# lmjakt/kmer_spans

Measured on AMD Instinct MI355X. Metric: Gbases/sec scanned (k=13, log-ratio score) at 1/2/4/8 MI355X; spans bit-exact, higher is better.
Workload: dtype f64

## Files before the change

kmer_spans_amd/csrc/ks_scan_chunked.hip:

```cpp
#include <hip/hip_fp16.h>
#include <hipcub/hipcub.hpp>

#include <algorithm>
#include <cstring>
#include <type_traits>
#include <vector>

#include "ks_scan_common.h"

namespace ks {

ks_status launch_scan_lane(ks_ctx *ctx, const uint8_t *seq, int64_t total, const int64_t *ra, const int64_t *rb,
                           const int32_t *rs, int64_t n, int k, const TableView &tv, uint64_t mw,
                           double min_score, uint32_t *visits, const RegionBuf &out,
                           const unsigned long long *d_cnt = nullptr, int64_t segcap = 0,
                           const ScanMode &mode = ScanMode(), int init_step = 1, const int64_t *offs = nullptr,
                           const uint32_t *packed = nullptr, hipStream_t strm = nullptr);

namespace {

constexpr int CH = 256;
constexpr int NB = 16;
constexpr int kModeClean = 0, kModeL = 1, kModeR = 2, kModeU = 3;

// ... 1434 lines not shown
  __shared__ __attribute__((aligned(16))) uint32_t s_esc[(BS / 64) * 2 * 64];
  __shared__ double s_lut[kLineLutMax];
  for (int i = threadIdx.x; i < tv.nlut; i += BS) s_lut[i] = tv.lut[i];
  __syncthreads();
  const int lane = threadIdx.x & 63, wv = threadIdx.x >> 6;
  const int64_t c = g.c0 + (int64_t)blockIdx.x * BS + threadIdx.x;
  if (c - lane >= g.nch) return;
  const bool live = c < g.nch;
  const int64_t start = live ? g.start[c] : (int64_t)k;
  const int n = live ? g.n[c] : 0;
  const bool first = live && (c == 0 || g.run[c - 1] != g.run[c]);
  const uint32_t kmask = (1u << (2 * k)) - 1u;
  P1Lane<!kExact, kTrlr, kExact> L;
  L.init(start, n, first, live, (live && xh) ? xh[c] : 0.0);
  LaneBases B;
  B.load(g.packed, total, start - k);
  const int kx = k + J - 1;
  const uint64_t xmask = (1ull << (2 * kx)) - 1ull;
  uint64_t x = B.first_key(kx);
  const double first_val = (kTrlr && first) ? ec.ks[(uint32_t)(x >> (2 * (J - 1))) & kmask] : 0.0;

  uint8_t *const ring = s_ring + wv * 4096;
  uint32_t *const esc = s_esc + wv * 128;
  const uint32_t ring_lds = __builtin_amdgcn_readfirstlane(lds_addr(ring));
  const uint32_t esc_lds = __builtin_amdgcn_readfirstlane(lds_addr(esc));
  const uint8_t *__restrict__ lines = tv.line;
  auto dwords = [&](uint64_t xk) -> uint32_t {
    const uint32_t c1 = (uint32_t)(xk >> 4) & 3u, c2 = (uint32_t)(xk >> 2) & 3u, c3 = (uint32_t)xk & 3u;
    const uint32_t d2 = (13u * (OWN + 4 + 4 * c1 + c2)) >> 5, d3 = (B3 + 11u * (16 * c1 + 4 * c2 + c3)) >> 5;
    return d2 | (d3 << 8);
  };
  auto issue = [&](uint64_t xk, int slot) {
    const uint32_t idx = (uint32_t)(xk >> 6), dd = dwords(xk);
    const int j = lane & 7;
#pragma unroll
    for (int q = 0; q < 8; ++q) {
      const int ow = 8 * q + (lane >> 3);
      const uint32_t li = (uint32_t)__shfl((int)idx, ow);
      const uint32_t od = (uint32_t)__shfl((int)dd, ow);
      const uint32_t d2 = od & 0xffu, d3 = od >> 8;
      const uint32_t dw = j < NO ? (uint32_t)j
                                 : (j < NO + 2 ? d2 + (uint32_t)(j - NO)
                                               : (j < NO + 4 ? min(d3 + (uint32_t)(j - NO - 2), 31u) : 0u));
      glds4(lines + (size_t)li * 128 + dw * 4, ring_lds + (uint32_t)(slot * 2048 + q * 256));
    }
  };
  double vp[J];
  uint64_t xp = 0;
  bool ep = false;
  constexpr int KW = kc_words(J);
  uint32_t *const kcl = kStore ? kc + kc_slot(live ? c : g.c0, 0, J) : nullptr;
  uint32_t recp[KW] = {};
  auto process = [&](int sp_, const double *vv, uint64_t xk, bool e) {
    double v5 = vv[J - 1];
    uint32_t c5 = 0;
    if (e) {
      const uint32_t pr = esc[(sp_ & 1) * 64 + lane];
      const uint32_t km = (uint32_t)xk & kmask;
      c5 = (km & 1u) ? (pr >> 16) : (pr & 0xffffu);
      v5 = s_lut[c5];
    }
    if constexpr (kStore) {
      uint32_t rec[KW];
#pragma unroll
      for (int q = 0; q < KW; ++q) rec[q] = recp[q];
      rec[(J - 1) / 2] |= c5 << (16 * ((J - 1) & 1));
      if (live) kc_store<KW>(kcl + (size_t)sp_ * 64 * KW, rec);
    }
#pragma unroll
    for (int t = 0; t < J; ++t) {
      const int i = sp_ * J + t;
      if (i < n) {
        double sv = t == J - 1 ? v5 : vv[t];
        if (kTrlr && first && i == 0) sv = first_val;
        if (visits) atomicAdd(&visits[(uint32_t)(xk >> (2 * (J - 1 - t))) & kmask], 1u);
        L.step(sv, i, ec, cand);
      }
    }
  };
  uint64_t x1 = 0, x2 = 0;
  issue(x, 0);
  x1 = B.next_key(x, J, xmask);
  issue(x1, 1);
  for (int st = 0; st < NS; ++st) {
    const uint64_t xs = x;
    if constexpr (kStore) {
      if (st + 1 >= NS) asm volatile("s_waitcnt vmcnt(1)" ::: "memory");
      else if (st >= 2) asm volatile("s_waitcnt vmcnt(9)" ::: "memory");
      else asm volatile("s_waitcnt vmcnt(8)" ::: "memory");
    } else {
      if (st + 1 < NS) asm volatile("s_waitcnt vmcnt(8)" ::: "memory");
      else asm volatile("s_waitcnt vmcnt(0)" ::: "memory");
    }
    const uint8_t *ln = ring + (st & 1) * 2048 + lane * 32;
    double v[J];
    uint32_t rec[KW] = {};
    bool e = false;
    {
      const uint4 q0 = *reinterpret_cast<const uint4 *>(ln);
      const uint4 q1 = *reinterpret_cast<const uint4 *>(ln + 16);
      const uint32_t D[8] = {q0.x, q0.y, q0.z, q0.w, q1.x, q1.y, q1.z, q1.w};
      const uint64_t lo = (uint64_t)D[0] | ((uint64_t)D[1] << 32);
      const uint64_t hi = (uint64_t)D[2] | (NO > 3 ? ((uint64_t)D[3] << 32) : 0ull);
      auto f13 = [&](int b) -> uint32_t {
        const uint64_t w = b < 64 ? ((lo >> b) | (b > 51 ? (hi << (64 - b)) : 0ull)) : (hi >> (b - 64));
        return (uint32_t)w & 0x1fffu;
      };
      const uint32_t c1 = (uint32_t)(xs >> 4) & 3u, c2 = (uint32_t)(xs >> 2) & 3u, c3 = (uint32_t)xs & 3u;
      uint32_t cs[J];
#pragma unroll
      for (int t = 0; t < OWN; ++t) cs[t] = f13(13 * t);
      const uint32_t l0 = f13(13 * OWN), l1 = f13(13 * (OWN + 1)), l2 = f13(13 * (OWN + 2)),
                     l3 = f13(13 * (OWN + 3));
      cs[OWN] = c1 == 0 ? l0 : (c1 == 1 ? l1 : (c1 == 2 ? l2 : l3));
      const uint32_t b2 = 13u * (OWN + 4 + 4 * c1 + c2), b3 = B3 + 11u * (16 * c1 + 4 * c2 + c3);
      cs[OWN + 1] = (uint32_t)(((uint64_t)D[NO] | ((uint64_t)D[NO + 1] << 32)) >> (b2 & 31)) & 0x1fffu;
      const uint32_t c11 = (uint32_t)(((uint64_t)D[NO + 2] | ((uint64_t)D[NO + 3] << 32)) >> (b3 & 31)) & 0x7ffu;
      e = c11 == 0x7ffu;
      cs[OWN + 2] = e ? 0u : c11;
#pragma unroll
      for (int t = 0; t < J; ++t) v[t] = s_lut[cs[t]];
      if constexpr (kStore) kc_pack<J>(cs, rec);
    }
    {
      const uint32_t km = (uint32_t)xs & kmask;
      const uint16_t *src = e ? tv.codes + (km & ~1u) : tv.codes;
      glds4(src, esc_lds + (uint32_t)((st & 1) * 256));
    }
    x = x1;
    if (st + 2 < NS) {
      x2 = B.next_key(x1, J, xmask);
      asm volatile("s_waitcnt lgkmcnt(0)" ::: "memory");
      issue(x2, st & 1);
      x1 = x2;
    }
    if (st > 0) process(st - 1, vp, xp, ep);
#pragma unroll
    for (int t = 0; t < J; ++t) vp[t] = v[t];
    if constexpr (kStore) {
#pragma unroll
      for (int q = 0; q < KW; ++q) recp[q] = rec[q];
    }
    xp = xs;
    ep = e;
  }
  if constexpr (kStore) asm volatile("s_waitcnt vmcnt(1)" ::: "memory");
  else asm volatile("s_waitcnt vmcnt(0)" ::: "memory");
  process(NS - 1, vp, xp, ep);
  if (!live) return;
  if constexpr (kExact) L.finish_exact(c, g, o, cr, xh, err);
  else L.finish(c, o, sp);
}

constexpr int kCodeBlock = 1024;
constexpr int kCodeDepth = 2;

__device__ __forceinline__ uint32_t packed_kmer(const uint32_t *__restrict__ packed, int64_t total, int64_t p0, int k) {
  const int64_t w0 = p0 >> 4, wlast = total >> 4;
  const uint64_t x = ((uint64_t)packed[min(w0, wlast)] << 32) | packed[min(w0 + 1, wlast)];
  const int sk = (int)(p0 & 15);
  return (uint32_t)(x >> (64 - 2 * (sk + k))) & ((1u << (2 * k)) - 1u);
}

template <int J, bool kTrlr, bool kVisits>
__global__ void __launch_bounds__(kCodeBlock) k_pass1c(Chunks g, int64_t total, int k, TableView tv, EmitCfg ec,
                                                       uint32_t *__restrict__ visits, P1 o, Cand cand,
                                                       const double *__restrict__ xh, Carry cr,
                                                       unsigned int *__restrict__ err,
                                                       const uint32_t *__restrict__ kc) {
  constexpr int NS = kc_steps(J), W = kc_words(J), D = kCodeDepth;
  constexpr int NG = (NS + D - 1) / D;
  extern __shared__ double s_clut[];
  for (int i = threadIdx.x; i < tv.nlut; i += kCodeBlock) s_clut[i] = tv.lut[i];
  __syncthreads();
  const int64_t c = g.c0 + (int64_t)blockIdx.x * kCodeBlock + threadIdx.x;
  if (c >= g.nch) return;
  const int64_t start = g.start[c];
  const int n = g.n[c];
  const bool first = c == 0 || g.run[c - 1] != g.run[c];
  const uint32_t kmask = (1u << (2 * k)) - 1u;
  const uint32_t *__restrict__ rp = kc + kc_slot(c, 0, J);
  uint32_t cur[D][W] = {}, nxt[D][W] = {};
  auto fetch = [&](int gi, uint32_t (&b)[D][W]) {
#pragma unroll
    for (int d = 0; d < D; ++d)
      if (gi * D + d < NS) kc_load<W>(rp + (size_t)(gi * D + d) * 64 * W, b[d]);
  };
  fetch(0, cur);
  P1Lane<false, kTrlr, true> L;
  L.init(start, n, first, true, xh[c]);
  double first_val = 0.0;
  if ((kTrlr && first) || (c & 63) == 0) {
    const uint32_t km0 = packed_kmer(g.packed, total, start - k, k);
    if (kTrlr && first) first_val = ec.ks[km0];
    if ((c & 63) == 0 && (cur[0][0] & 0xffffu) != (uint32_t)tv.codes[km0]) atomicOr(err, 128u);
  }
  LaneBases B;
  uint64_t x = 0;
  const uint64_t xmask = (1ull << (2 * (k + J - 1))) - 1ull;
  if (kVisits) {
    B.load(g.packed, total, start - k);
    x = B.first_key(k + J - 1);
  }
  for (int gi = 0; gi < NG; ++gi) {
    if (gi + 1 < NG) fetch(gi + 1, nxt);
    if (gi * D * J < n) {
#pragma unroll
      for (int d = 0; d < D; ++d) {
        const int st = gi * D + d;
        if (st < NS) {
#pragma unroll
          for (int t = 0; t < J; ++t) {
            const int i = st * J + t;
            if (i < n) {
              const uint32_t code = (cur[d][t >> 1] >> (16 * (t & 1))) & 0xffffu;
              double sv = s_clut[code];
              if (kTrlr && first && i == 0) sv = first_val;
              if (kVisits) atomicAdd(&visits[(uint32_t)(x >> (2 * (J - 1 - t))) & kmask], 1u);
              L.step(sv, i, ec, cand);
            }
          }
          if (kVisits) x = B.next_key(x, J, xmask);
        }
      }
    }
#pragma unroll
    for (int d = 0; d < D; ++d)
#pragma unroll
      for (int q = 0; q < W; ++q) cur[d][q] = nxt[d][q];
  }
  L.finish_exact(c, g, o, cr, xh, err);
}

__global__ void __launch_bounds__(256) k_test_codes(uint32_t *__restrict__ kc, Chunks g, Carry cr, int64_t nch,
                                                    int J, int what, unsigned int *__restrict__ err) {
  auto spoil = [&](int64_t c, int i) {
    uint32_t *p = kc + kc_slot(c, i / J, J) + (size_t)((i % J) >> 1);
    const int sh = 16 * ((i % J) & 1);
    const uint32_t code = (*p >> sh) & 0xffffu;
    *p = (*p & ~(0xffffu << sh)) | ((code ? 0u : 1u) << sh);
  };
  if (what == 1) {
    for (int64_t c = threadIdx.x; c < nch; c += blockDim.x)
      for (int i = 0; i < CH; ++i) spoil(c, i);
  } else if (what == 0) {
    if (threadIdx.x == 0) spoil(0, 0);
  } else {
    __shared__ unsigned long long s_first;
    if (threadIdx.x == 0) s_first = ~0ull;
    __syncthreads();
    for (int64_t c = threadIdx.x; c < nch; c += blockDim.x)
      if ((c & 63) != 0 && g.n[c] > 1 && c + 1 < nch && g.run[c + 1] == g.run[c] && cr.mode[c] != kModeClean &&
          cr.hq[c] < 0)
        atomicMin(&s_first, (unsigned long long)c);
    __syncthreads();
    if (threadIdx.x == 0) {
      if (s_first == ~0ull) atomicOr(err, 256u);
      else spoil((int64_t)s_first, 1);
    }
  }
}

constexpr int kRankBlock = 768;

template <int OWN>
__global__ void __launch_bounds__(kRankBlock) k_pass1r(Chunks g, int64_t total, int k, TableView tv, EmitCfg ec,
                                                       uint32_t *__restrict__ visits, P1 o, Cand cand) {
  constexpr int BS = kRankBlock;
  constexpr int J = OWN + 2;
  constexpr int NS = (CH + J - 1) / J;
  static_assert(OWN + 2 <= 8, "own, L1, L2 dwords in 8 lanes");
  __shared__ __attribute__((aligned(16))) uint8_t s_ring[(BS / 64) * 2 * 2048];
  __shared__ unsigned long long s_pc[2 * kRankPieceLds];
  const int nl = min(tv.nrpc, kRankPieceLds);
  for (int i = threadIdx.x; i < 2 * nl; i += BS) s_pc[i] = tv.rpc[i];
  __syncthreads();
  const int lane = threadIdx.x & 63, wv = threadIdx.x >> 6;
  const int64_t c = g.c0 + (int64_t)blockIdx.x * BS + threadIdx.x;
  if (c - lane >= g.nch) return;
  const bool live = c < g.nch;
  const int64_t start = live ? g.start[c] : (int64_t)k;
  const int n = live ? g.n[c] : 0;
  const bool first = live && (c == 0 || g.run[c - 1] != g.run[c]);
  const uint32_t kmask = (1u << (2 * k)) - 1u;
  P1Lane<false, false> L;
  L.init(start, n, first, live, 0.0);
  LaneBases B;
  B.load(g.packed, total, start - k);
  const int kx = k + J - 1;
  const uint64_t xmask = (1ull << (2 * kx)) - 1ull;
  uint64_t x = B.first_key(kx);
  uint8_t *const ring = s_ring + wv * 4096;
  const uint32_t ring_lds = __builtin_amdgcn_readfirstlane(lds_addr(ring));
  const uint8_t *__restrict__ lines = tv.rline;
  const unsigned long long *__restrict__ gpc = tv.rpc;
  const double thr = tv.rthr;
  auto issue = [&](uint64_t xk, int slot) {
    const uint32_t idx = (uint32_t)(xk >> 4);
    const uint32_t c1 = (uint32_t)(xk >> 2) & 3u, c2 = (uint32_t)xk & 3u;
    const uint32_t dd = (OWN + c1) | ((OWN + 4 + 4 * c1 + c2) << 8);
    const int j = lane & 7;
#pragma unroll
    for (int q = 0; q < 8; ++q) {
      const int ow = 8 * q + (lane >> 3);
      const uint32_t li = (uint32_t)__shfl((int)idx, ow);
      const uint32_t od = (uint32_t)__shfl((int)dd, ow);
      const uint32_t dw = j < OWN ? (uint32_t)j : (j == OWN ? (od & 0xffu) : (j == OWN + 1 ? (od >> 8) : 0u));
      glds4(lines + (size_t)li * 128 + dw * 4, ring_lds + (uint32_t)(slot * 2048 + q * 256));
    }
  };
  auto decode = [&](uint32_t code) -> double {
    const uint32_t p = code >> kRankOffBits;
    const unsigned long long off = code & ((1u << kRankOffBits) - 1u);
    unsigned long long base, inc;
    if ((int)p < nl) {
      base = s_pc[2 * p];
      inc = s_pc[2 * p + 1];
    } else {
      base = gpc[2 * p];
      inc = gpc[2 * p + 1];
    }
    return __longlong_as_double((long long)(base + off * inc)) - thr;
  };
  double vp[J];
  uint64_t xp = 0;
  auto process = [&](int sp_, const double *vv, uint64_t xk) {
#pragma unroll
    for (int t = 0; t < J; ++t) {
      const int i = sp_ * J + t;
      if (i < n) {
        if (visits) atomicAdd(&visits[(uint32_t)(xk >> (2 * (J - 1 - t))) & kmask], 1u);
        L.step(vv[t], i, ec, cand);
      }
    }
  };
  uint64_t x1 = 0, x2 = 0;
  issue(x, 0);
  x1 = B.next_key(x, J, xmask);
  issue(x1, 1);
  for (int st = 0; st < NS; ++st) {
    const uint64_t xs = x;
    if (st + 1 < NS) asm volatile("s_waitcnt vmcnt(8)" ::: "memory");
    else asm volatile("s_waitcnt vmcnt(0)" ::: "memory");
    const uint8_t *ln = ring + (st & 1) * 2048 + lane * 32;
    uint32_t cs[J];
    {
      const uint4 q0 = *reinterpret_cast<const uint4 *>(ln);
      const uint4 q1 = *reinterpret_cast<const uint4 *>(ln + 16);
      const uint32_t D[8] = {q0.x, q0.y, q0.z, q0.w, q1.x, q1.y, q1.z, q1.w};
#pragma unroll
      for (int t = 0; t < J; ++t) cs[t] = D[t];
    }
    x = x1;
    if (st + 2 < NS) {
      x2 = B.next_key(x1, J, xmask);
      asm volatile("s_waitcnt lgkmcnt(0)" ::: "memory");
      issue(x2, st & 1);
      x1 = x2;
    }
    if (st > 0) process(st - 1, vp, xp);
#pragma unroll
    for (int t = 0; t < J; ++t) vp[t] = decode(cs[t]);
    xp = xs;
  }
  asm volatile("s_waitcnt vmcnt(0)" ::: "memory");
  process(NS - 1, vp, xp);
  if (live) L.finish(c, o, SummP1{});
}

constexpr int kLdsTableK = 7;
__global__ void __launch_bounds__(1024) k_pass1_lds_int(Chunks g, int64_t total, int k, TableView tv, EmitCfg ec,
                                                        uint32_t *__restrict__ visits, P1 o, Cand cand) {
  __shared__ int32_t s_val[1 << (2 * kLdsTableK)];
  const int nk = 1 << (2 * k);
  for (int i = threadIdx.x; i < nk; i += blockDim.x) s_val[i] = (int32_t)tv_get(tv, (uint32_t)i);
  __syncthreads();
  const uint32_t kmask = (uint32_t)nk - 1u;
  for (int64_t c = g.c0 + (int64_t)blockIdx.x * blockDim.x + threadIdx.x; c < g.nch;
       c += (int64_t)gridDim.x * blockDim.x) {
    const int64_t start = g.start[c];
    const int n = g.n[c];
    const int64_t q0 = start - k;
    Window16 win(g.packed, total, q0);
    int32_t prev = 0, best = 0, asum = 0, pmin = INT32_MAX, pmax = INT32_MIN;
    int beg = -1, arg = 0, parg = 0;
// ... 1960 lines not shown
  int32_t *se = cv.take<int32_t>(nch);
  long long *sD = cv.take<long long>(nch * 6);
  int32_t *sA = cv.take<int32_t>(nch * 2);
  double *x = cv.take<double>(nch);
  uint8_t *cmode = cv.take<uint8_t>(nch);
  int32_t *hq = cv.take<int32_t>(nch * 2);
  double *hmax = cv.take<double>(nch);
  unsigned long long *cnts = cv.take<unsigned long long>(5 * kSegs + 8);
  uint8_t *flag = cv.take<uint8_t>(nch + 64);
  char *xa0 = cv.take<char>(ntiles * 32), *xa1 = cv.take<char>(ntiles * 32);
  double *pa = cv.take<double>(nch);
  double *pb = cv.take<double>(nch);
  uint8_t *pz = cv.take<uint8_t>(nch);
  int32_t *spe = cv.take<int32_t>(nch * 2);
  long long *spd = cv.take<long long>(nch * 6);
  int32_t *spa = cv.take<int32_t>(nch * 2);
  unsigned long long *nfix = cv.take<unsigned long long>(nch + 2);
  uint8_t *ssel = cv.take<uint8_t>(nch);
  double2 *tagg = cv.take<double2>(ntiles);
  double *tin = cv.take<double>(ntiles);
  const int64_t ngt = nch / 64 + 2;
  int32_t *gte = cv.take<int32_t>(ngt);
  long long *gtd = cv.take<long long>(ngt * 6);
  long long *gtm = cv.take<long long>(ngt);
  int32_t *gtee = cv.take<int32_t>(ngt);
  const int64_t rcap_h = std::max<int64_t>(65536, nch / 128);
  int32_t *rslot = cv.take<int32_t>(nch);
  int64_t *rchunk = cv.take<int64_t>(2 * rcap_h);
  unsigned long long *rcnt = cv.take<unsigned long long>(8);
  double *rval = cv.take<double>(2 * rcap_h * 256);
  *bytes = cv.off;

  Work w{};
  if (!base) return w;
  w.g = Chunks{kp.start, kp.n, kp.run, nch, packed};
  w.p1 = P1{p1d, p1d + nch, p1d + 2 * nch, p1d + 3 * nch, p1d + 4 * nch, p1d + 5 * nch, p1i, p1i + nch, spec,
            p1i + 2 * nch};
  w.p1.ep = ep;
  w.sm = Summ{se, sD, sD + 2 * nch, sD + 4 * nch, sA};
  w.cr = Carry{x, cmode, hq, hmax, hq + nch};
  w.cnts = cnts;
  w.flag = flag;
  auto xtiles = [&](char *p) {
    return XTiles{reinterpret_cast<int32_t *>(p), reinterpret_cast<int32_t *>(p) + ntiles,
                  reinterpret_cast<long long *>(p + ntiles * 8), reinterpret_cast<long long *>(p + ntiles * 16),
                  reinterpret_cast<double *>(p + ntiles * 24)};
  };
  w.xagg = xtiles(xa0);
  w.xtin = xtiles(xa1);
  w.pa = pa;
  w.pb = pb;
  w.pz = pz;
  w.sp1 = SummP1{spe, spd, spd + 2 * nch, spd + 4 * nch, spa};
  w.nfix = nfix;
  w.fix = reinterpret_cast<int64_t *>(nfix + 2);
  w.tagg = tagg;
  w.tin = tin;
  w.trun = kp.trun;
  w.tcomp = TileComp{gte, gtd, gtd + 2 * ngt, gtd + 4 * ngt, gtm, gtee};
  w.rpb = ReplayBuf{plan.p1summ ? rslot : nullptr, rchunk, rval, rcnt, rcap_h};
  if (plan.p1summ) {
    w.sm.sel = ssel;
    w.sm.pD = w.sp1.D;
    w.sm.pM = w.sp1.M;
    w.sm.pN = w.sp1.N;
    w.sm.pA = w.sp1.A;
  }
  w.nwin = (nch + 63) / 64;
  return w;
}

struct ScanCall {
  ks_ctx *ctx;
  const ks_dev_seqs *s;
  int64_t total;
  int k;
  const TableView &tv;
  const EmitCfg ec;
  const Runs &runs;
  const RunLayout &lay;
  const RegionBuf &rb;
  uint32_t *visits, *visits_rescan;
  const ScanMode &mode;
};

Chunks view(const Chunks &g, const Half &h) {
  Chunks v = g;
  v.c0 = h.c0;
  v.nch = h.c1;
  return v;
}

constexpr int kWpb = 2;

ks_status ascan(const ScanCall &c, const Work &w, const P1 &o, double *out, const Half &h, hipStream_t strm) {
  const int64_t nruns = c.runs.n;
  if (h.r1 <= h.r0) return KS_OK;
  const dim3 gr((unsigned)(h.r1 - h.r0));
  if (h.t1 <= h.t0) return launch(k_approx_scan, gr, dim3(64), 0, strm, c.lay.cbase, h.r1, o, out, h.r0);
  const dim3 g4((unsigned)((h.t1 - h.t0 + kWpb - 1) / kWpb)), b4(64 * kWpb);
  KS_TRY(launch(k_ascan_tiles, g4, b4, 0, strm, c.lay.tbase, c.lay.cbase, nruns, w.trun, o, w.tagg, h.t0, h.t1));
  KS_TRY(launch(k_ascan_runs, gr, dim3(64), 0, strm, c.lay.tbase, h.r1, w.tagg, w.tin, h.r0));
  return launch(k_ascan_apply, g4, b4, 0, strm, c.lay.tbase, c.lay.cbase, nruns, w.trun, o, w.tin, out, h.t0, h.t1);
}

ks_status predict(const ScanCall &c, const Work &w, const Half &h, hipStream_t strm) {
  P1 pp = w.p1;
  pp.asum = w.pa;
  pp.cexit = w.pb;
  pp.special = w.pz;
  KS_HIP(hipMemsetAsync(w.pz + h.c0, 0, (size_t)(h.c1 - h.c0), strm));
  const size_t lds = (size_t)2 << (2 * c.tv.approx_k);
  const int per_cu = lds <= ((size_t)32 << 10) ? 4 : 1;
  const unsigned gl = (unsigned)std::max<int64_t>(
      1, std::min<int64_t>((h.c1 - h.c0 + 1023) / 1024, (int64_t)c.ctx->num_cus * per_cu));
  KS_HIP(hipFuncSetAttribute((const void *)k_predict<4>, hipFuncAttributeMaxDynamicSharedMemorySize, (int)lds));
  KS_TRY(launch(k_predict<4>, dim3(gl), dim3(1024), lds, strm, view(w.g, h), c.total, c.k, c.tv.approx,
                c.tv.approx_k, pp.asum, pp.cexit));
  return ascan(c, w, pp, w.xh, h, strm);
}

ks_status pass1_half(const ScanCall &c, const ScanPlan &plan, const Work &w, const Half &h, hipStream_t strm,
                     const Cand &cand) {
  const Chunks gv = view(w.g, h);
  const int64_t n = h.c1 - h.c0;
  const TableView &tv = c.tv;
  const EmitCfg &ec = c.ec;
  const P1 &p1 = w.p1;
  const SummP1 &sp1 = w.sp1;
  const double *xh = plan.entry_reuse ? w.cr.x : (plan.p1summ ? w.xh : nullptr);
  const Carry &cr = w.cr;
  unsigned int *err = reinterpret_cast<unsigned int *>(w.cnts + 2 * kSegs + 2 * (&h - plan.half) + 1);
  const bool trlr = ec.trlr != 0;
  auto blocks = [&](int64_t per) { return dim3((unsigned)((n + per - 1) / per)); };
  auto persistent = [&](int per_cu) {
    return dim3((unsigned)std::max<int64_t>(1, std::min<int64_t>((n + 1023) / 1024, (int64_t)per_cu * c.ctx->num_cus)));
  };
  switch (plan.family) {
    case P1Family::Lds:
      if (trlr)
        return launch(k_pass1_lds<true>, persistent(1), dim3(1024), 0, strm, gv, c.total, c.k, tv, ec, c.visits, p1,
                      cand, xh, sp1);
      if (plan.exact)
        return launch(k_pass1_lds_int, persistent(2), dim3(1024), 0, strm, gv, c.total, c.k, tv, ec, c.visits, p1,
                      cand);
      return launch(k_pass1_lds<false>, persistent(1), dim3(1024), 0, strm, gv, c.total, c.k, tv, ec, c.visits, p1,
                    cand, xh, sp1);
    case P1Family::Line: {
      const int own = tv.line_own;
      if (plan.codes_read)
        return pick_int<5, 7, 4>(plan.codes_J, [&](auto j) {
          return pick_bool(trlr, [&](auto t) {
            return pick_bool(c.visits != nullptr, [&](auto v) {
              return launch(k_pass1c<decltype(j)::value, decltype(t)::value, decltype(v)::value>, blocks(kCodeBlock),
                            dim3(kCodeBlock), (size_t)tv.nlut * 8, strm, gv, c.total, c.k, tv, ec, c.visits, p1, cand,
                            xh, cr, err, w.kc);
            });
          });
        });
      if (tv.rline && !trlr && !plan.p1summ && own == 3)
        return launch(k_pass1r<3>, blocks(kRankBlock), dim3(kRankBlock), 0, strm, gv, c.total, c.k, tv, ec, c.visits,
                      p1, cand);
      if (tv.line_kind == 3)
        return pick_wide_own(own, [&](auto o) {
          return pick_bool(trlr, [&](auto t) {
            return pick_int<1, 2, 0>(plan.entry_reuse ? (plan.codes_write ? 2 : 1) : 0, [&](auto x) {
              return launch(k_pass1w<decltype(o)::value, decltype(t)::value, (decltype(x)::value > 0),
                                     (decltype(x)::value > 1)>,
                            blocks(kWideBlock), dim3(kWideBlock), 0, strm, gv, c.total, c.k, tv, ec, c.visits, p1, cand,
                            xh, sp1, cr, err, w.kc);
            });
          });
        });
      if (!plan.comp)
        return pick_int<3, 4, 2>(own, [&](auto o) {
          return pick_bool(trlr, [&](auto t) {
            return launch(k_pass1l<decltype(o)::value, true, false, decltype(t)::value>, blocks(1024), dim3(1024), 0,
                          strm, gv, c.total, c.k, tv, ec, c.visits, p1, cand, xh, sp1, cr, err, w.kc);
          });
        });
      return pick_u16_own(own, [&](auto o) {
        return pick_bool(tv.nlut <= kLineLutMax, [&](auto l) {
          return pick_bool(trlr, [&](auto t) {
            return pick_int<1, 2, 0>(plan.entry_reuse ? (plan.codes_write ? 2 : 1) : 0, [&](auto x) {
              return launch(k_pass1l<decltype(o)::value, false, decltype(l)::value, decltype(t)::value,
                                     (decltype(x)::value > 0), (decltype(x)::value > 1 && decltype(l)::value)>,
                            blocks(768), dim3(768), 0, strm, gv, c.total, c.k, tv, ec, c.visits, p1, cand, xh, sp1, cr,
                            err, w.kc);
            });
          });
        });
      });
    }
    case P1Family::F64Expanded:
      return pick_int<3, 4, 2>(plan.J, [&](auto j) {
        return pick_bool(trlr, [&](auto t) {
          return launch(k_pass1pf<decltype(j)::value, decltype(t)::value, 512>, blocks(512), dim3(512), 0, strm, gv,
                        c.s->seq, c.total, c.k, tv, ec, c.visits, p1, cand, c.runs.packed, xh, sp1);
        });
      });
    case P1Family::CompExpanded:
      return pick_int<3, 5, 2>(plan.J, [&](auto j) {
        return pick_bool(plan.lds_lut, [&](auto l) {
          return pick_bool(trlr, [&](auto t) {
            return launch(k_pass1p<decltype(j)::value, decltype(l)::value, decltype(t)::value>, blocks(kP1Block),
                          dim3(kP1Block), 0, strm, gv, c.s->seq, c.total, c.k, tv, ec, c.visits, p1, cand,
                          c.runs.packed, xh, sp1);
          });
        });
      });
    case P1Family::Plain:
      break;
  }
  return fail(KS_ERR_INTERNAL, "chunked scan: no pass-1 launch per half for this table form");
}

ks_status pass1_tail(const ScanCall &c, const ScanPlan &plan, const Work &w, hipStream_t strm, const Cand &cand) {
  const dim3 grid((unsigned)((w.g.nch - plan.ctail + 1023) / 1024));
  auto go = [&](auto j, auto comp, auto l) {
    return launch(k_pass1<decltype(j)::value, decltype(comp)::value, decltype(l)::value>, grid, dim3(1024), 0, strm,
                  w.g, c.s->seq, c.total, c.k, c.tv, nullptr, c.ec, c.visits, w.p1, cand, plan.ctail, 1);
  };
  if (plan.family == P1Family::F64Expanded)
    return pick_int<3, 4, 2>(plan.J, [&](auto j) { return go(j, std::false_type{}, std::false_type{}); });
  if (plan.J == 5) return go(std::integral_constant<int, 5>{}, std::true_type{}, std::false_type{});
  return pick_int<3, 4, 2>(plan.J, [&](auto j) {
    return pick_bool(plan.lds_lut, [&](auto l) { return go(j, std::true_type{}, l); });
  });
}

ks_status post_half(const ScanCall &c, const ScanPlan &plan, const Work &w, int hi, hipStream_t strm) {
  const Half &h = plan.half[hi];
  const bool last = hi == plan.nhalf - 1;
  const Chunks gv = view(w.g, h);
  const Chunks &g = w.g;
  const TableView &tv = c.tv;
  const P1 &p1 = w.p1;
  const Summ &sm = w.sm;
  const Carry &cr = w.cr;
  const TileComp &tch = w.tcomp;
  const ReplayBuf &rpb = w.rpb;
  const uint8_t *seq = c.s->seq;
  const int64_t total = c.total, nruns = c.runs.n;
  const int k = c.k;
  const int64_t nh = h.c1 - h.c0, nr = h.r1 - h.r0, nt = h.t1 - h.t0;
  if (nh <= 0) return KS_OK;
  unsigned long long *rep_h = w.cnts + 2 * kSegs + 2 * hi;
  unsigned int *err_h = reinterpret_cast<unsigned int *>(rep_h + 1);
  const dim3 gch_h((unsigned)((nh + 255) / 256)), gsum_h((unsigned)((nh + 1023) / 1024));
  const dim3 bw(64 * kWpb);
  const dim3 gst((unsigned)((nt + kWpb - 1) / kWpb));
  auto stitch = [&]() -> ks_status {
    if (nt > 0)
      KS_TRY(launch(k_stitch_tiles, gst, bw, 0, strm, g, c.lay.tbase, c.lay.cbase, nruns, w.trun, p1, cr, w.xagg, h.t0,
                    h.t1));
    if (nr > 0)
      KS_TRY(launch(k_stitch_runs, dim3((unsigned)nr), dim3(64), 0, strm, c.lay.tbase, h.r1, c.runs.a, c.runs.b,
                    c.runs.seq, c.ec, w.xagg, w.xtin, c.rb, w.rss[hi], h.r0));
    if (nt > 0)
      KS_TRY(launch(k_stitch_emit, gst, bw, 0, strm, g, c.lay.tbase, c.lay.cbase, nruns, w.trun, c.runs.a, c.runs.seq,
                    p1, cr, c.ec, w.xtin, c.rb, w.rss[hi], err_h, h.t0, h.t1));
    return KS_OK;
  };
  if (plan.entry_reuse) {
    if (last) {
      KS_HIP(hipEventRecord(c.ctx->ev[kEvP2End], strm));
      KS_HIP(hipEventRecord(c.ctx->ev[kEvP34End], strm));
    }
    return stitch();
  }
  KS_TRY(ascan(c, w, p1, w.xt, h, strm));
  const int64_t wl = (h.c0 > 0 ? h.c0 - 1 : 0) / 64;
  const int64_t nwm = (h.c1 + 63) / 64 - wl;
  if (plan.exact) {
    KS_TRY(launch(k_carry_exact, gch_h, dim3(256), 0, strm, gv, p1, w.xt, cr));
  } else if (plan.p1summ) {
    KS_HIP(hipMemsetAsync(w.nfix + hi, 0, 8, strm));
    KS_HIP(hipMemsetAsync(rpb.count + hi, 0, 8, strm));
    KS_TRY(launch(k_marks_select, dim3((unsigned)((nwm + 3) / 4)), dim3(256), 0, strm, gv, p1, w.xt, w.flag, nwm,
                  w.sp1, sm, w.fix + h.c0, w.nfix + hi, w.xh,
                  w.dbg ? reinterpret_cast<unsigned long long *>(w.dbg + w.nwin * 9) : nullptr, rpb, hi));
    const unsigned gw = (unsigned)std::max<int64_t>(1, (int64_t)c.ctx->num_cus * 8);
    KS_TRY(launch(k_summ_fixw<false>, dim3(gw), dim3(256), 0, strm, g, seq, total, k, tv, w.xt, w.fix + h.c0,
                  w.nfix + hi, sm, rpb, hi));
  } else {
    KS_TRY(launch(k_seg_marks, dim3((unsigned)((nwm + kWpb - 1) / kWpb)), bw, 0, strm, gv, p1, w.xt, w.flag, nwm));
    if (plan.no_summ) {
      KS_TRY(launch(k_summ_none, gsum_h, dim3(1024), 0, strm, gv, sm));
    } else if (plan.lds_table) {
      if (plan.comp && plan.lds_lut) {
        const size_t tb = (size_t)2 << (2 * k);
        KS_HIP(hipFuncSetAttribute((const void *)k_summaries<true, true, true>,
                                   hipFuncAttributeMaxDynamicSharedMemorySize, (int)tb));
        KS_TRY(launch(k_summaries<true, true, true>, gsum_h, dim3(1024), tb, strm, gv, seq, total, k, tv, nullptr, p1,
                      w.xt, sm));
      } else {
        const size_t tb = (size_t)8 << (2 * k);
        KS_HIP(hipFuncSetAttribute((const void *)k_summaries<false, false, true>,
                                   hipFuncAttributeMaxDynamicSharedMemorySize, (int)tb));
        KS_TRY(launch(k_summaries<false, false, true>, gsum_h, dim3(1024), tb, strm, gv, seq, total, k, tv, nullptr,
                      p1, w.xt, sm));
      }
    } else if (plan.lds_lut) {
      KS_TRY(launch(k_summaries<true, true>, gsum_h, dim3(1024), 0, strm, gv, seq, total, k, tv, w.codes, p1, w.xt,
                    sm));
    } else if (plan.comp) {
      KS_TRY(launch(k_summaries<true, false>, gsum_h, dim3(1024), 0, strm, gv, seq, total, k, tv, w.codes, p1, w.xt,
                    sm));
// ... 543 lines not shown
```

Before: 1016.

## Specialize code-read pass1 for full chunks with inlined branchless scoring step

For the no-visits path, the code-read pass-1 kernel now walks chunks with a compile-time split between full wavefronts (all chunks length CH), where per-element bounds checks are dropped, and a partial path that keeps them. The generic lane step is replaced by an inlined branchless routine that updates the head and span state directly. Per-value special-value classification is skipped when the LUT has no non-finite entries, detected with a block-wide OR during the LUT load. The block size for this variant drops from 1024 to 768 to allow more registers per thread. The cost is duplicated scoring logic that must stay bit-exact with the original lane step, plus larger code.

```diff
diff --git a/kmer_spans_amd/csrc/ks_scan_chunked.hip b/kmer_spans_amd/csrc/ks_scan_chunked.hip
--- a/kmer_spans_amd/csrc/ks_scan_chunked.hip
+++ b/kmer_spans_amd/csrc/ks_scan_chunked.hip
@@ -1610,7 +1610,7 @@
   else L.finish(c, o, sp);
 }
 
-constexpr int kCodeBlock = 1024;
+constexpr int code_block(bool visits) { return visits ? 1024 : 768; }
 constexpr int kCodeDepth = 2;
 
 __device__ __forceinline__ uint32_t packed_kmer(const uint32_t *__restrict__ packed, int64_t total, int64_t p0, int k) {
@@ -1620,26 +1620,72 @@
   return (uint32_t)(x >> (64 - 2 * (sk + k))) & ((1u << (2 * k)) - 1u);
 }
 
+template <bool kTrlr>
+__device__ __forceinline__ void code_index(P1Lane<false, kTrlr, true> &L, bool &pos, bool &act, double s, int i,
+                                           const EmitCfg &ec, int reach, const Cand &cand, bool classify) {
+  {
+    Head &h = L.hx;
+    const double t = h.T + s;
+    const bool tp = t > 0;
+    const double T = tp ? t : 0.0;
+    const bool hup = act & tp & (T > h.hmax);
+    h.hq = (act & !tp) ? i : h.hq;
+    h.hmax = hup ? T : h.hmax;
+    h.harg = hup ? i : h.harg;
+    h.T = T;
+    act = act & tp;
+  }
+  if (classify) L.special |= !isfinite(s);
+  const double tt = L.prev + s;
+  const bool pn = tt > 0;
+  const double S = pn ? tt : 0.0;
+  const bool open = !pos & pn;
+  const bool close = pos & !pn;
+  if (kTrlr ? (close & (i - L.beg >= reach)) : (close & (L.best >= ec.min_score))) {
+    const int f0 = L.f0, arg = L.arg, beg = L.beg;
+    const long long ml = kTrlr ? ec.min_len : 0;
+    const bool want =
+        kTrlr ? ((((long long)((arg != f0 ? arg - 1 : arg) - (beg != f0 ? beg - 1 : beg)) >= ml) |
+                  ((long long)((i != f0 ? i - 1 : i) - (arg != f0 ? arg - 1 : arg) - 1) >= (ml > 1 ? ml : 1LL))))
+              : ((uint64_t)(int64_t)(arg - beg) >= ec.mw);
+    if (want) cand_put(cand, L.start, beg, arg, i, L.best);
+  }
+  const bool up = open | (S > L.best);
+  L.best = up ? S : L.best;
+  L.arg = up ? i : L.arg;
+  L.beg = open ? i : L.beg;
+  L.prev = S;
+  pos = pn;
+}
+
+#define KS_INLINE_LAMBDA __attribute__((always_inline))
 template <int J, bool kTrlr, bool kVisits>
-__global__ void __launch_bounds__(kCodeBlock) k_pass1c(Chunks g, int64_t total, int k, TableView tv, EmitCfg ec,
+__global__ void __launch_bounds__(code_block(kVisits)) k_pass1c(Chunks g, int64_t total, int k, TableView tv, EmitCfg ec,
                                                        uint32_t *__restrict__ visits, P1 o, Cand cand,
                                                        const double *__restrict__ xh, Carry cr,
                                                        unsigned int *__restrict__ err,
                                                        const uint32_t *__restrict__ kc) {
   constexpr int NS = kc_steps(J), W = kc_words(J), D = kCodeDepth;
   constexpr int NG = (NS + D - 1) / D;
+  constexpr int kCodeBlock = code_block(kVisits);
+  constexpr int LAST = CH - (NS - 1) * J;
+  static_assert((NG - 1) * D < NS && LAST >= 1 && LAST <= J, "only the last batch is short, only the last step partial");
   extern __shared__ double s_clut[];
-  for (int i = threadIdx.x; i < tv.nlut; i += kCodeBlock) s_clut[i] = tv.lut[i];
-  __syncthreads();
+  int bad = 0;
+  for (int i = threadIdx.x; i < tv.nlut; i += kCodeBlock) {
+    const double v = tv.lut[i];
+    s_clut[i] = v;
+    if (!kVisits) bad |= !isfinite(v);
+  }
+  const bool lut_special = kVisits ? (__syncthreads(), false) : __syncthreads_or(bad) != 0;
   const int64_t c = g.c0 + (int64_t)blockIdx.x * kCodeBlock + threadIdx.x;
   if (c >= g.nch) return;
   const int64_t start = g.start[c];
   const int n = g.n[c];
   const bool first = c == 0 || g.run[c - 1] != g.run[c];
-  const uint32_t kmask = (1u << (2 * k)) - 1u;
   const uint32_t *__restrict__ rp = kc + kc_slot(c, 0, J);
   uint32_t cur[D][W] = {}, nxt[D][W] = {};
-  auto fetch = [&](int gi, uint32_t (&b)[D][W]) {
+  auto fetch = [&](int gi, uint32_t (&b)[D][W]) KS_INLINE_LAMBDA {
 #pragma unroll
     for (int d = 0; d < D; ++d)
       if (gi * D + d < NS) kc_load<W>(rp + (size_t)(gi * D + d) * 64 * W, b[d]);
@@ -1653,42 +1699,104 @@
     if (kTrlr && first) first_val = ec.ks[km0];
     if ((c & 63) == 0 && (cur[0][0] & 0xffffu) != (uint32_t)tv.codes[km0]) atomicOr(err, 128u);
   }
-  LaneBases B;
-  uint64_t x = 0;
-  const uint64_t xmask = (1ull << (2 * (k + J - 1))) - 1ull;
-  if (kVisits) {
+  if (!kVisits && kTrlr && first && n > 0) L.special = !isfinite(first_val);
+  const long long rl = kTrlr ? (long long)ec.min_len - 1 : 0;
+  const int reach = (int)(rl < 0 ? 0 : (rl > CH ? CH + 1 : rl));
+  using std::integral_constant;
+  using std::true_type;
+  using std::false_type;
+  auto step = [&](auto full, auto live, int st, const uint32_t (&r)[W]) KS_INLINE_LAMBDA {
+    constexpr bool kFull = decltype(full)::value;
+    constexpr int LIVE = decltype(live)::value;
+    auto value = [&](int t) KS_INLINE_LAMBDA { return s_clut[(r[t >> 1] >> (16 * (t & 1))) & 0xffffu]; };
+    double v[LIVE];
+    if (kFull) {
+#pragma unroll
+      for (int t = 0; t < LIVE; ++t) v[t] = value(t);
+      if (kTrlr) v[0] = (first && st == 0) ? first_val : v[0];
+    }
+    bool pos = L.prev > 0, act = L.hx.hq < 0;
+#pragma unroll
+    for (int t = 0; t < LIVE; ++t) {
+      const int i = st * J + t;
+      if (kFull || i < n) {
+        double sv;
+        if (kFull) {
+          sv = v[t];
+        } else {
+          sv = value(t);
+          if (kTrlr && first && i == 0) sv = first_val;
+        }
+        code_index<kTrlr>(L, pos, act, sv, i, ec, reach, cand, lut_special);
+      }
+    }
+  };
+  auto walk = [&](bool full) KS_INLINE_LAMBDA {
+    auto either = [&](auto live, int st, const uint32_t (&r)[W]) KS_INLINE_LAMBDA {
+      if (full) step(true_type{}, live, st, r);
+      else step(false_type{}, live, st, r);
+    };
+    for (int gi = 0; gi < NG - 1; ++gi) {
+      fetch(gi + 1, nxt);
+      if (full || gi * D * J < n) {
+#pragma unroll
+        for (int d = 0; d < D; ++d) either(integral_constant<int, J>{}, gi * D + d, cur[d]);
+      }
+#pragma unroll
+      for (int d = 0; d < D; ++d)
+#pragma unroll
+        for (int q = 0; q < W; ++q) cur[d][q] = nxt[d][q];
+    }
+    if (full || (NG - 1) * D * J < n) {
+      auto rest = [&](auto self, auto dc) KS_INLINE_LAMBDA {
+        constexpr int d = decltype(dc)::value, st = (NG - 1) * D + d;
+        if constexpr (st < NS) {
+          either(integral_constant<int, (st == NS - 1 ? LAST : J)>{}, st, cur[d]);
+          self(self, integral_constant<int, d + 1>{});
+        }
+      };
+      rest(rest, integral_constant<int, 0>{});
+    }
+  };
+  if constexpr (kVisits) {
+    LaneBases B;
+    const uint32_t kmask = (1u << (2 * k)) - 1u;
+    const uint64_t xmask = (1ull << (2 * (k + J - 1))) - 1ull;
     B.load(g.packed, total, start - k);
-    x = B.first_key(k + J - 1);
-  }
-  for (int gi = 0; gi < NG; ++gi) {
-    if (gi + 1 < NG) fetch(gi + 1, nxt);
-    if (gi * D * J < n) {
-#pragma unroll
-      for (int d = 0; d < D; ++d) {
-        const int st = gi * D + d;
-        if (st < NS) {
-#pragma unroll
-          for (int t = 0; t < J; ++t) {
-            const int i = st * J + t;
-            if (i < n) {
-              const uint32_t code = (cur[d][t >> 1] >> (16 * (t & 1))) & 0xffffu;
-              double sv = s_clut[code];
-              if (kTrlr && first && i == 0) sv = first_val;
-              if (kVisits) atomicAdd(&visits[(uint32_t)(x >> (2 * (J - 1 - t))) & kmask], 1u);
-              L.step(sv, i, ec, cand);
+    uint64_t x = B.first_key(k + J - 1);
+    for (int gi = 0; gi < NG; ++gi) {
+      if (gi + 1 < NG) fetch(gi + 1, nxt);
+      if (gi * D * J < n) {
+#pragma unroll
+        for (int d = 0; d < D; ++d) {
+          const int st = gi * D + d;
+          if (st < NS) {
+#pragma unroll
+            for (int t = 0; t < J; ++t) {
+              const int i = st * J + t;
+              if (i < n) {
+                const uint32_t code = (cur[d][t >> 1] >> (16 * (t & 1))) & 0xffffu;
+                double sv = s_clut[code];
+                if (kTrlr && first && i == 0) sv = first_val;
+                atomicAdd(&visits[(uint32_t)(x >> (2 * (J - 1 - t))) & kmask], 1u);
+                L.step(sv, i, ec, cand);
+              }
             }
+            x = B.next_key(x, J, xmask);
           }
-          if (kVisits) x = B.next_key(x, J, xmask);
         }
       }
-    }
-#pragma unroll
-    for (int d = 0; d < D; ++d)
-#pragma unroll
-      for (int q = 0; q < W; ++q) cur[d][q] = nxt[d][q];
+#pragma unroll
+      for (int d = 0; d < D; ++d)
+#pragma unroll
+        for (int q = 0; q < W; ++q) cur[d][q] = nxt[d][q];
+    }
+  } else {
+    walk(__ballot(n == CH) == ~0ull);
   }
   L.finish_exact(c, g, o, cr, xh, err);
 }
+#undef KS_INLINE_LAMBDA
 
 __global__ void __launch_bounds__(256) k_test_codes(uint32_t *__restrict__ kc, Chunks g, Carry cr, int64_t nch,
                                                     int J, int what, unsigned int *__restrict__ err) {
@@ -3955,8 +4063,9 @@
         return pick_int<5, 7, 4>(plan.codes_J, [&](auto j) {
           return pick_bool(trlr, [&](auto t) {
             return pick_bool(c.visits != nullptr, [&](auto v) {
-              return launch(k_pass1c<decltype(j)::value, decltype(t)::value, decltype(v)::value>, blocks(kCodeBlock),
-                            dim3(kCodeBlock), (size_t)tv.nlut * 8, strm, gv, c.total, c.k, tv, ec, c.visits, p1, cand,
+              constexpr int kBlock = code_block(decltype(v)::value);
+              return launch(k_pass1c<decltype(j)::value, decltype(t)::value, decltype(v)::value>, blocks(kBlock),
+                            dim3(kBlock), (size_t)tv.nlut * 8, strm, gv, c.total, c.k, tv, ec, c.visits, p1, cand,
                             xh, cr, err, w.kc);
             });
           });
```

Measured after the change: 1090 (median of 6 runs). +7.3%, better.
